# JackShDr/InfluentialRS

Hardware: AMD Instinct MI355X
Metric: scored user-item pairs/sec (whole node) (higher is better)
Workload: dtype f32; 1 GPU; c2: n_item=3415, d=128, L=200, H=4, layers=6, ffn=256; one greedy path-search step; users_per_gpu=4096, top_k=100, sweep=bf16 filter + exact f32 re-score, parallelism=single GPU

## Files before the change

### influentialrs_amd/csrc/decoder.hip

```cpp
#include "irs_internal.h"
#include "plane_split.h"

#include <assert.h>

typedef __attribute__((ext_vector_type(16))) float f32x16;

__global__ void __launch_bounds__(256) k_embed(const int64_t *__restrict__ seq, const float *__restrict__ E,
                                               const float *__restrict__ pe, float *__restrict__ x, int rows, int L,
                                               int d, float sqrtd, int64_t n_item) {
    int row = blockIdx.x * 4 + (threadIdx.x >> 6);
    int lane = threadIdx.x & 63;
    if (row >= rows) return;
    int64_t id = seq[row];
    if (id < 0) id = 0;
    if (id > n_item) id = n_item;
    int t = row % L;
    const float *e = E + id * (int64_t)d;
    const float *p = pe + (int64_t)t * d;
    float *o = x + (int64_t)row * d;
    for (int c = lane; c < d; c += 64) o[c] = __fadd_rn(__fmul_rn(e[c], sqrtd), p[c]);
}

__global__ void k_pif(const int64_t *__restrict__ user, const float *__restrict__ U, const float *__restrict__ w,
                      const float *__restrict__ b, float *__restrict__ r_u, int B, int ud, int64_t n_user) {
// ... 1386 lines not shown
    return;
#endif
#pragma unroll
    for (int j = 0; j < 8; ++j) {
        const float v = t[8 * s + j];
        const __bf16 h = (__bf16)v;
        const float r1 = v - (float)h;
        const __bf16 m = (__bf16)r1;
        const float r2 = r1 - (float)m;
        X[0][j] = h;
        X[1][j] = m;
        X[2][j] = (__bf16)r2;
    }
}

template <int B_, int E_, class Fn>
__device__ __forceinline__ void x6_static_for(Fn &&fn) {
    if constexpr (B_ < E_) {
        fn(std::integral_constant<int, B_>{});
        x6_static_for<B_ + 1, E_>(fn);
    }
}
template <int OFF>
__device__ __forceinline__ x6_u32x4 x6_rd(unsigned int base) {
    x6_u32x4 v;
    asm volatile("ds_read_b128 %0, %1 offset:%2" : "=v"(v) : "v"(base), "i"(OFF));
    return v;
}

template <int OFF>
__device__ __forceinline__ x6_u32x4 x6_gld(const void *p) {
    x6_u32x4 v;
    asm volatile("global_load_dwordx4 %0, %1, off offset:%2" : "=v"(v) : "v"(p), "i"(OFF) : "memory");
    return v;
}

__device__ __forceinline__ unsigned int x6_gld32(const void *p) {
    unsigned int v;
    asm volatile("global_load_dword %0, %1, off" : "=v"(v) : "v"(p) : "memory");
    return v;
}

__device__ __forceinline__ unsigned int x6_gld32_sync(const void *p) {
    unsigned int v;
    asm volatile("global_load_dword %0, %1, off\n\ts_waitcnt vmcnt(0)" : "=v"(v) : "v"(p) : "memory");
    return v;
}

template <int OFF>
__device__ __forceinline__ void x6_gst(void *p, x6_u32x4 v) {
    asm volatile("global_store_dwordx4 %0, %1, off offset:%2" :: "v"(p), "v"(v), "i"(OFF) : "memory");
}

template <int OFF>
__device__ __forceinline__ void x6_wr64(unsigned int addr, __attribute__((ext_vector_type(4))) _Float16 v) {
    asm volatile("ds_write_b64 %0, %1 offset:%2" :: "v"(addr), "v"(v), "i"(OFF));
}

template <int OFF>
__device__ __forceinline__ x6_u32x4 x6_rd_sync(unsigned int base) {
    x6_u32x4 v;
    asm volatile("ds_read_b128 %0, %1 offset:%2\n\ts_waitcnt lgkmcnt(0)" : "=v"(v) : "v"(base), "i"(OFF));
    return v;
}

struct SeqTarget {
    int seq;
    float k[8], v[8];
};
__device__ __forceinline__ unsigned int seq_diag_mask(int L, int qb, bool tgt, int pq) {
    unsigned int pm = 0;
    const int k0_ = 16 * qb;
    if (L <= k0_) return 0;
    if (L - k0_ < 16) pm = (0xFFFFu << (L - k0_)) & 0xFFFFu;
    if (tgt && L - 1 >= k0_ && L - 1 < k0_ + 16) pm |= 1u << (L - 1 - k0_);
    if (pq >= k0_ && pq < k0_ + 16) pm |= 1u << (pq - k0_);
    return pm;
}
__device__ __forceinline__ void seq_attn_block(const float *Ks, const char *Vp, int PL, int L, int qb, unsigned int pm_diag, float tgt_add,
                                               bool tgt_ok, int pq, const float *qscr, float4 *of, bool store, int seq, SeqTarget &tg);
#ifndef SEQ_EXP
#define SEQ_EXP 0
#endif
#define X6_SEQ_VECS (256 + 12 * 32 * 4 + 384)
#define X6_SEQ_KIMG (3 * 16384 + X6_SEQ_VECS * 4)
#define X6_SEQ_VIMG (X6_SEQ_KIMG + 32768)
#define X6_SEQ_SCR (X6_SEQ_VIMG + 32768)
#define X6_SEQ_SCR_B 4608
__host__ __device__ constexpr int x6_seq_lds_bytes() { return X6_SEQ_SCR + 8 * X6_SEQ_SCR_B; }
#ifdef X6_STAMP
#define X6_T(v_) { unsigned long long t_; asm volatile("s_memtime %0\n\ts_waitcnt lgkmcnt(0)" : "=s"(t_) :: "memory"); v_ = t_; }
#if X6_STAMP + 0 == 2
#define X6_TI(v_)
#else
#define X6_TI(v_) X6_T(v_)
#endif
#define X6_PH(i_) { unsigned long long t_; asm volatile("s_memtime %0\n\ts_waitcnt lgkmcnt(0)" : "=s"(t_) :: "memory"); st_ph[i_] += t_ - st_prev; st_prev = t_; }
#else
#define X6_T(v_)
#define X6_TI(v_)
#define X6_PH(i_)
#endif
template <int QP0, int NW, bool EMBED, int NT = 4, int NPL = 3, bool SEQ = false>
__global__ void __launch_bounds__(64 * NW, (NT == 8 || NW == 8) ? 1 : 2) k_block_x6(BlockX6Args a) {
    static_assert(!SEQ || (NT == 4 && NPL == 2 && NW == 8 && !EMBED && QP0 == 3), "the sequence-resident form: d = 128, float16 planes, eight waves, no q | k | v tail");
    constexpr int NP = 8 * NPL, STEP_B = x6_step_b(NPL);
    using x6_plane = typename std::conditional<NPL == 2, x6_f16x8, x6_bf16x8>::type;
    constexpr int D = 32 * NT, F = 256, NSLOT = SEQ ? 3 : x6_nslot(NPL), LEAD = NSLOT - 1, PPW = NP / NW, HT = NT / 4;
    constexpr int NFRONT = SEQ ? 3 * NT : 0;
    constexpr float WS = x6_wscale(NPL), IWS = 1.0f / WS;
    constexpr bool RESID_LATE = NPL == 2 && NT == 4 && !EMBED && NSLOT == 4 && (NW == 4 || NW == 8);
    constexpr bool RESID_SEP = RESID_LATE || SEQ;
    constexpr int NLOAD = 4 * NT;
    constexpr int NPRE = x6_npre(NT), NOUT = NT * HT;
    constexpr int S0 = EMBED ? NPRE : 0;
    constexpr int V_B1 = 0, V_B2 = F, V_G = F + D, V_B = F + 2 * D, V_BIN = F + 3 * D, V_O = F + 3 * D + 3 * D;
    constexpr int V_BQ = V_O + 6 * D;
    static_assert(NT == 4 || NT == 8, "d = 128 or 256");
    extern __shared__ __attribute__((aligned(16))) char smem[];
    float *vecs = reinterpret_cast<float *>(smem + NSLOT * STEP_B);
    const int tid = threadIdx.x;
    const int lane = tid & 63, wave = __builtin_amdgcn_readfirstlane(tid >> 6);
    const int li = lane & 31, lk = lane >> 5;
    unsigned long long st_p[8] = {0, 0, 0, 0, 0, 0, 0, 0};
    X6_T(st_p[0])
    const int m0 = blockIdx.x * (32 * NW);
    const int M = SEQ ? 0x7FFFFFFF : (a.m_dev ? min(a.M, a.m_dev[0]) : a.M);
    int sh_b[2] = {-1, -1}, sh_qb[2] = {0, 0}, sh_cnt[2] = {0, 0}, sh_pq[2] = {-1, -1}, sh_row0[2] = {0, 0};
    int sh_off[2] = {0, 0};
    float sh_ru[2] = {0.f, 0.f};
    bool sh_tgt[2] = {false, false};
    unsigned int sh_pm[2] = {0, 0};
    float sh_tadd[2] = {0.f, 0.f};
    if constexpr (SEQ) {
        if ((int)blockIdx.x >= a.n_wg_dev[0]) return;
        const int tg_ = blockIdx.x * NW + wave;
        const bool irn_ = a.mask_mode == IRS_MASK_IRN;
#pragma unroll
        for (int h = 0; h < 2; ++h) {
            const int b_ = __builtin_amdgcn_readfirstlane(a.tile_seq[2 * tg_ + h]);
            sh_b[h] = b_;
            if (b_ >= 0) {
                sh_qb[h] = __builtin_amdgcn_readfirstlane(a.tile_qb[2 * tg_ + h]);
                const int off_ = __builtin_amdgcn_readfirstlane(a.seq_off[b_]);
                sh_off[h] = off_;
                sh_cnt[h] = __builtin_amdgcn_readfirstlane(a.seq_cnt[b_]);
                sh_pq[h] = __builtin_amdgcn_readfirstlane(a.seq_padq[b_]), sh_row0[h] = __builtin_amdgcn_readfirstlane(a.seq_row0[b_]);
                sh_ru[h] = irn_ ? a.r_u[b_] : 0.f;
                sh_tgt[h] = irn_ && a.seq[(int64_t)b_ * a.L + a.L - 1] != 0;
                sh_pm[h] = seq_diag_mask(sh_cnt[h], sh_qb[h], sh_tgt[h], sh_pq[h]);
                sh_tadd[h] = __builtin_bit_cast(float, __builtin_amdgcn_readfirstlane(__builtin_bit_cast(int, irn_ ? (1.0f - sh_ru[h]) * 1.4426950408889634f : 0.f)));
            }
        }
    }
    float pv[RESID_LATE ? 13 : 1];
    if constexpr (RESID_LATE) {
        const int td = tid & (D - 1);
        const float *pbo = a.bo ? a.bo : a.b2, *pc = a.c ? a.c : a.b2, *pg2 = a.c ? a.g2 : a.b2, *pb2n = a.c ? a.b2n : a.b2;
        pv[0] = a.b1[tid], pv[1] = a.bin[tid], pv[2] = a.bin[256 + td], pv[3] = a.b2[td], pv[4] = a.g[td], pv[5] = a.b[td];
        pv[6] = pbo[td], pv[7] = a.g1[td], pv[8] = a.b1n[td], pv[9] = pc[td], pv[10] = pg2[td], pv[11] = pb2n[td];
        pv[12] = 0.f;
    }
    if (!SEQ && m0 >= M) return;
    if constexpr (RESID_LATE) {
        static_assert(NW == 4 || NW == 8, "every thread index below 256 exists");
        asm volatile("" ::"v"(pv[0]), "v"(pv[1]), "v"(pv[2]), "v"(pv[3]), "v"(pv[4]), "v"(pv[5]), "v"(pv[6]), "v"(pv[7]), "v"(pv[8]),
                     "v"(pv[9]), "v"(pv[10]), "v"(pv[11]));
        if (tid < 256) {
            vecs[V_B1 + tid] = pv[0];
            vecs[V_BIN + tid] = pv[1];
        }
        if (tid < D) {
            vecs[V_BIN + 256 + tid] = pv[2];
            vecs[V_B2 + tid] = pv[3], vecs[V_G + tid] = pv[4], vecs[V_B + tid] = pv[5];
            vecs[V_O + 0 * D + tid] = a.bo ? pv[6] : 0.f;
            vecs[V_O + 1 * D + tid] = pv[7];
            vecs[V_O + 2 * D + tid] = pv[8];
            vecs[V_O + 3 * D + tid] = a.c ? pv[9] : 0.f;
            vecs[V_O + 4 * D + tid] = a.c ? pv[10] : 0.f;
            vecs[V_O + 5 * D + tid] = a.c ? pv[11] : 0.f;
        }
    } else if constexpr (NT == 4) {
        if constexpr (SEQ) {
            constexpr int NV_ = (X6_SEQ_VECS + 64 * NW - 1) / (64 * NW);
// ... 200 lines not shown
#pragma unroll
            for (int tn = 0; tn < NT; ++tn)
#pragma unroll
                for (int g = 0; g < 4; ++g) {
                    const float4 t4 = rfrag[(tn * 4 + g) * 64];
                    acc[tn][4 * g + 0] = t4.x * WS, acc[tn][4 * g + 1] = t4.y * WS, acc[tn][4 * g + 2] = t4.z * WS, acc[tn][4 * g + 3] = t4.w * WS;
                }
        }
        if constexpr (RESID_LATE) {
            x6_static_for<0, NT>([&](auto tc) __attribute__((always_inline)) {
                constexpr int tn = decltype(tc)::value;
                const float4 *tp = afrag + tn * 4 * 64;
                atq[tn][0] = x6_gld<0>(tp), atq[tn][1] = x6_gld<1024>(tp), atq[tn][2] = x6_gld<2048>(tp), atq[tn][3] = x6_gld<3072>(tp);
            });
        } else if constexpr (!SEQ) {
#pragma unroll
            for (int tn = 0; tn < NT; ++tn)
#pragma unroll
                for (int g = 0; g < 4; ++g) {
                    const float4 t4 = afrag[(tn * 4 + g) * 64];
                    at[tn][4 * g + 0] = t4.x, at[tn][4 * g + 1] = t4.y, at[tn][4 * g + 2] = t4.z, at[tn][4 * g + 3] = t4.w;
                }
        }
        if constexpr (RESID_LATE) {
#pragma unroll
            for (int tn = 0; tn < NT; ++tn)
#pragma unroll
                for (int r = 0; r < 16; ++r) acc[tn][r] = 0.f;
        }
    } else {
        const int l31 = lane & 31, lhi = lane >> 5;
        char *scr = smem + wave * 16384;
        float4 *xo = reinterpret_cast<float4 *>(a.Xf) + fbase;
        int64_t rid[16];
        int rpos[16];
#pragma unroll
        for (int i = 0; i < 16; ++i) {
            const int mr = m0 + wave * 32 + 2 * i + lhi;
            const int orig = mr < M ? (a.tok_row ? a.tok_row[mr] : mr) : 0;
            int64_t id = mr < M ? a.seq[orig] : 0;
            if (id < 0) id = 0;
            if (id > a.n_item) id = a.n_item;
            rid[i] = id, rpos[i] = orig % a.L;
        }
#pragma unroll
        for (int hf = 0; hf < NT / 4; ++hf) {
            float4 ev[16], pv[16];
#pragma unroll
            for (int i = 0; i < 16; ++i) {
                ev[i] = *reinterpret_cast<const float4 *>(a.E + rid[i] * (int64_t)D + 128 * hf + 4 * l31);
                pv[i] = *reinterpret_cast<const float4 *>(a.pe + (int64_t)rpos[i] * D + 128 * hf + 4 * l31);
            }
#pragma unroll
            for (int i = 0; i < 16; ++i) {
                const int r = 2 * i + lhi;
                const bool live = m0 + wave * 32 + r < M;
                float4 v = make_float4(0.f, 0.f, 0.f, 0.f);
                if (live)
                    v = make_float4(__fadd_rn(__fmul_rn(ev[i].x, a.sqrtd), pv[i].x), __fadd_rn(__fmul_rn(ev[i].y, a.sqrtd), pv[i].y),
                                    __fadd_rn(__fmul_rn(ev[i].z, a.sqrtd), pv[i].z), __fadd_rn(__fmul_rn(ev[i].w, a.sqrtd), pv[i].w));
                *reinterpret_cast<float4 *>(scr + r * 512 + ((l31 ^ r) << 4)) = v;
            }
#pragma unroll
            for (int t4 = 0; t4 < 4; ++t4)
#pragma unroll
                for (int g = 0; g < 4; ++g) {
                    const int tn = 4 * hf + t4, c = 8 * t4 + 2 * g + lk;
                    const float4 v = *reinterpret_cast<const float4 *>(scr + li * 512 + ((c ^ li) << 4));
                    xo[(tn * 4 + g) * 64] = v;
                    acc[tn][4 * g + 0] = v.x, acc[tn][4 * g + 1] = v.y, acc[tn][4 * g + 2] = v.z, acc[tn][4 * g + 3] = v.w;
                }
        }
        __syncthreads();
    }
    auto load_res = [&]() __attribute__((always_inline)) {
        if constexpr (RESID_SEP) {
            const float4 *rfrag = reinterpret_cast<const float4 *>(a.Rf) + fbase;
            x6_static_for<0, NT>([&](auto tc) __attribute__((always_inline)) {
                constexpr int tn = decltype(tc)::value;
                const float4 *tp = rfrag + tn * 4 * 64;
                resq[tn][0] = x6_gld<0>(tp), resq[tn][1] = x6_gld<1024>(tp), resq[tn][2] = x6_gld<2048>(tp), resq[tn][3] = x6_gld<3072>(tp);
            });
        }
    };
    if constexpr (RESID_LATE) {
        asm volatile("s_waitcnt vmcnt(%0) lgkmcnt(0)" :: "i"(PPW * (LEAD - 1) + NLOAD) : "memory");
        __builtin_amdgcn_s_barrier();
    } else {
        issue(S0);
        asm volatile("s_waitcnt vmcnt(0) lgkmcnt(0)" ::: "memory");
        __builtin_amdgcn_s_barrier();
        x6_static_for<1, LEAD>([&](auto ic) __attribute__((always_inline)) { issue(S0 + decltype(ic)::value); });
    }

    constexpr int RING = 4, RA = RING - 1;
    static_assert(NP % RING == 0 && (NP + 8) % RING == 0 && RA <= NP / 2, "ring index continuity; next-step reads stay behind the barrier");
    x6_u32x4 af[RING];
    auto landed_all = [&]() __attribute__((always_inline)) {
#pragma unroll
        for (int q = 0; q < RING; ++q) asm volatile("s_waitcnt lgkmcnt(0)" : "+v"(af[q]));
    };
    x6_static_for<0, RING>([&](auto qc) __attribute__((always_inline)) {
        constexpr int q = decltype(qc)::value, off = (S0 % NSLOT) * STEP_B + (q < RA ? q : RA - 1) * 1024;
        if constexpr (NT == 8) af[q] = x6_rd_sync<off>(fr_addr);
        else af[q] = x6_rd<off>(fr_addr);
    });
    if constexpr (NT != 8) landed_all();

    auto seq_sync_tail = [&](int i) __attribute__((always_inline)) {
        return (i < NFRONT && i % 3 == 2) || i == NFRONT + NOUT - 1 || i == NFRONT + NPRE - 1;
    };
    const float invn = 1.0f / (float)D;
    x6_plane X[NPL];
    unsigned long long st_a = 0, st_b = 0, st_c = 0, st_d = 0, st_wait = 0, st_bar = 0, st_iss = 0, st_0 = 0, st_1 = 0, st_steps = 0;
    X6_T(st_0)
#ifdef X6_NO_MFMA
#define X6_MM(W_, X_, T_) { const auto mw_ = (W_); const auto mx_ = (X_); asm volatile("" :: "v"(mw_), "v"(mx_)); }
#else
#define X6_MM(W_, X_, T_) T_ = x6_mma(W_, X_, T_)
#endif
#define X6_MFMA(Wreg, Xp, T_) X6_MM(__builtin_bit_cast(x6_plane, Wreg), X[Xp], T_)
#ifdef X6_DUMP
#define X6_DUMP_FRAG(I_, f_) if (blockIdx.x == 0 && wave == 0) a.dbg[((I_) * NP + (f_)) * 64 + lane] = __builtin_bit_cast(uint4, af[(f_) & RA]);
#else
#define X6_DUMP_FRAG(I_, f_)
#endif
#ifdef X6_NO_READS
#define X6_READ_AHEAD(f_) asm volatile("" : "+v"(af[(f_) & RA]));
#else
#define X6_READ_AHEAD(f_)                                                                                                \
    if constexpr ((f_) + RA < NP) af[((f_) + RA) & RA] = x6_rd<((f_) + RA) * 1024>(sb_);                                 \
    else if (SEQ && !(SEQ_EXP & 2) && seq_sync_tail(step_)) af[((f_) + RA) & RA] = x6_rd_sync<((f_) + RA - NP) * 1024>(sn_);  \
    else af[((f_) + RA) & RA] = x6_rd<((f_) + RA - NP) * 1024>(sn_);  \
    asm volatile("s_waitcnt lgkmcnt(%1)" : "+v"(af[(f_) & RA]) : "i"(RA));                                               \
    X6_DUMP_FRAG(step_, f_)
#endif
#ifdef X6_NO_DMA
#define X6_ISSUE(i_)
#else
#define X6_ISSUE(i_) issue(i_)
#endif
#ifdef X6_NO_BARRIER
#define X6_PUBLISH(I_) if ((I_) + LEAD < nsteps) X6_ISSUE((I_) + LEAD);
#else
#define X6_PUBLISH(I_)                                                                                                   \
    if ((I_) + 1 < nsteps) {                                                                                             \
        X6_TI(st_a)                                                                                                       \
        if (RESID_LATE && (I_) < 4) asm volatile("s_waitcnt vmcnt(%0)" :: "i"(PPW * (LEAD - 2) + NLOAD) : "memory");  \
        else if (LEAD > 2 && (I_) + 2 < nsteps) asm volatile("s_waitcnt vmcnt(%0)" :: "i"(PPW * (LEAD - 2)) : "memory");      \
        else asm volatile("s_waitcnt vmcnt(0)" ::: "memory");                                                            \
        X6_TI(st_b)                                                                                                       \
        __builtin_amdgcn_s_barrier();                                                                                    \
        X6_TI(st_c)                                                                                                       \
        if ((I_) + LEAD < nsteps && !(SEQ && (I_) == NFRONT + NPRE - 1 && end_rt))  \
            X6_ISSUE((I_) + LEAD);                                                                                        \
        if constexpr (RESID_LATE) { if ((I_) == 1) load_res(); }                                                         \
        X6_TI(st_d)                                                                                                       \
        st_wait += st_b - st_a, st_bar += st_c - st_b, st_iss += st_d - st_c;                                            \
        if (SEQ && (I_) < NFRONT && (I_) % 3 == 0) st_ph[10] += st_c - st_b;  \
        if (SEQ && (I_) == NFRONT) st_ph[11] += st_c - st_b;                  \
    }
#endif
#define X6_STEP(I_, SRC, T0, T1, T2, T3)                                                                                \
    {                                                                                                                    \
        const int step_ = (I_);                                                                                          \
        unsigned long long sq_0 = 0, sq_1 = 0;                                                                           \
        X6_TI(sq_0)                                                                                                       \
        const unsigned int sb_ = fr_addr + (unsigned int)((step_ % NSLOT) * STEP_B);                                     \
        const unsigned int sn_ = fr_addr + (unsigned int)(((step_ + 1) % NSLOT) * STEP_B);                               \
        x6_static_for<0, NP>([&](auto fc_) __attribute__((always_inline)) {                                              \
            constexpr int f_ = decltype(fc_)::value, g_ = f_ / NPL, pl_ = f_ % NPL;                                      \
            if constexpr (f_ == 0) x6_split(SRC, 0, X);                                                                  \
            if constexpr (f_ == NP / 2) {                                                                                \
                X6_PUBLISH(step_)                                                                                        \
                x6_split(SRC, 1, X);                                                                                     \
            }                                                                                                            \
            X6_READ_AHEAD(f_)                                                                                            \
            f32x16 &T_ = (g_ & 3) == 0 ? T0 : (g_ & 3) == 1 ? T1 : (g_ & 3) == 2 ? T2 : T3;                              \
             \
            x6_static_for<0, NPL - pl_>([&](auto qc_) __attribute__((always_inline)) {                                   \
                X6_MFMA(af[f_ & RA], NPL - 1 - pl_ - decltype(qc_)::value, T_);                                           \
            });                                                                                                          \
        });                                                                                                              \
        X6_TI(sq_1)                                                                                                       \
        st_steps += sq_1 - sq_0;                                                                                         \
        __builtin_amdgcn_sched_barrier(0);                                                                               \
    }

    auto vec_stream = [&](auto na_c, auto o0_c, auto o1_c, auto o2_c, auto &&use) __attribute__((always_inline)) {
        constexpr int NA = decltype(na_c)::value, O0 = decltype(o0_c)::value, O1 = decltype(o1_c)::value, O2 = decltype(o2_c)::value;
        constexpr int NG = 4 * NT, AH = NA == 1 ? 3 : 2, RG = AH + 1;
        x6_u32x4 pr[RG][NA];
        auto rd = [&](auto gc) __attribute__((always_inline)) {
            constexpr int gi = decltype(gc)::value, goff = ((gi >> 2) * 32 + (gi & 3) * 8) * 4;
            pr[gi % RG][0] = x6_rd<O0 * 4 + goff>(vecs_addr);
            if constexpr (NA > 1) pr[gi % RG][1] = x6_rd<O1 * 4 + goff>(vecs_addr);
            if constexpr (NA > 2) pr[gi % RG][2] = x6_rd<O2 * 4 + goff>(vecs_addr);
        };
        x6_static_for<0, AH>(rd);
        x6_static_for<0, NG>([&](auto gc) __attribute__((always_inline)) {
            constexpr int gi = decltype(gc)::value, newer = NA * (gi + AH < NG ? AH : NG - 1 - gi);
            if constexpr (gi + AH < NG) rd(std::integral_constant<int, gi + AH>{});
            if constexpr (NA == 1) asm volatile("s_waitcnt lgkmcnt(%1)" : "+v"(pr[gi % RG][0]) : "i"(newer));
            if constexpr (NA == 2) asm volatile("s_waitcnt lgkmcnt(%2)" : "+v"(pr[gi % RG][0]), "+v"(pr[gi % RG][1]) : "i"(newer));
            if constexpr (NA == 3) asm volatile("s_waitcnt lgkmcnt(%3)" : "+v"(pr[gi % RG][0]), "+v"(pr[gi % RG][1]), "+v"(pr[gi % RG][2]) : "i"(newer));
            use(gc, __builtin_bit_cast(float4, pr[gi % RG][0]), __builtin_bit_cast(float4, pr[gi % RG][NA > 1 ? 1 : 0]),
                __builtin_bit_cast(float4, pr[gi % RG][NA > 2 ? 2 : 0]));
        });
    };
    constexpr bool ASM_VECS = NT == 4;
    using x6_ic0 = std::integral_constant<int, 0>;
    auto layer_norm = [&](auto vb_c, auto vg_c, auto vbeta_c, auto vadd_c) __attribute__((always_inline)) {
        constexpr int vb = decltype(vb_c)::value, vg = decltype(vg_c)::value, vbeta = decltype(vbeta_c)::value, vadd = decltype(vadd_c)::value;
        float sum = 0.f;
        if constexpr (ASM_VECS && vb >= 0) {
            vec_stream(std::integral_constant<int, 1>{}, vb_c, x6_ic0{}, x6_ic0{}, [&](auto gc, const float4 bb, const float4, const float4) __attribute__((always_inline)) {
                constexpr int tn = decltype(gc)::value >> 2, g = decltype(gc)::value & 3;
                if constexpr (RESID_SEP) {
                    const float4 rs = __builtin_bit_cast(float4, resq[tn][g]);
                    acc[tn][4 * g + 0] = __builtin_fmaf(acc[tn][4 * g + 0], IWS, rs.x), acc[tn][4 * g + 1] = __builtin_fmaf(acc[tn][4 * g + 1], IWS, rs.y);
                    acc[tn][4 * g + 2] = __builtin_fmaf(acc[tn][4 * g + 2], IWS, rs.z), acc[tn][4 * g + 3] = __builtin_fmaf(acc[tn][4 * g + 3], IWS, rs.w);
                    acc[tn][4 * g + 0] += bb.x, acc[tn][4 * g + 1] += bb.y, acc[tn][4 * g + 2] += bb.z, acc[tn][4 * g + 3] += bb.w;
                } else {
                    acc[tn][4 * g + 0] = __builtin_fmaf(acc[tn][4 * g + 0], IWS, bb.x), acc[tn][4 * g + 1] = __builtin_fmaf(acc[tn][4 * g + 1], IWS, bb.y);
                    acc[tn][4 * g + 2] = __builtin_fmaf(acc[tn][4 * g + 2], IWS, bb.z), acc[tn][4 * g + 3] = __builtin_fmaf(acc[tn][4 * g + 3], IWS, bb.w);
                }
                sum += (acc[tn][4 * g + 0] + acc[tn][4 * g + 1]) + (acc[tn][4 * g + 2] + acc[tn][4 * g + 3]);
            });
        } else {
#pragma unroll
            for (int tn = 0; tn < NT; ++tn)
#pragma unroll
                for (int g = 0; g < 4; ++g) {
                    if constexpr (vb >= 0) {
                        const float4 bb = *reinterpret_cast<const float4 *>(vecs + vb + tn * 32 + 8 * g + 4 * lk);
                        acc[tn][4 * g + 0] = __builtin_fmaf(acc[tn][4 * g + 0], IWS, bb.x), acc[tn][4 * g + 1] = __builtin_fmaf(acc[tn][4 * g + 1], IWS, bb.y);
                        acc[tn][4 * g + 2] = __builtin_fmaf(acc[tn][4 * g + 2], IWS, bb.z), acc[tn][4 * g + 3] = __builtin_fmaf(acc[tn][4 * g + 3], IWS, bb.w);
                    }
                    sum += (acc[tn][4 * g + 0] + acc[tn][4 * g + 1]) + (acc[tn][4 * g + 2] + acc[tn][4 * g + 3]);
                    if constexpr (!ASM_VECS) __builtin_amdgcn_sched_barrier(0);
                }
        }
        const float mu = lanes_sum<32>(sum) * invn;
        float qs = 0.f;
#pragma unroll
        for (int tn = 0; tn < NT; ++tn)
#pragma unroll
            for (int r = 0; r < 16; ++r) {
                const float dlt = acc[tn][r] - mu;
                qs += dlt * dlt;
            }
        const float rstd = 1.0f / sqrtf(lanes_sum<32>(qs) * invn + 1e-5f);
        if constexpr (ASM_VECS) {
            auto norm = [&](auto gc, const float4 gg, const float4 be, const float4 ad_) __attribute__((always_inline)) {
                constexpr int tn = decltype(gc)::value >> 2, g = decltype(gc)::value & 3;
                const float4 ad = vadd >= 0 ? ad_ : make_float4(0.f, 0.f, 0.f, 0.f);
                acc[tn][4 * g + 0] = (acc[tn][4 * g + 0] - mu) * rstd * gg.x + be.x + ad.x;
                acc[tn][4 * g + 1] = (acc[tn][4 * g + 1] - mu) * rstd * gg.y + be.y + ad.y;
                acc[tn][4 * g + 2] = (acc[tn][4 * g + 2] - mu) * rstd * gg.z + be.z + ad.z;
                acc[tn][4 * g + 3] = (acc[tn][4 * g + 3] - mu) * rstd * gg.w + be.w + ad.w;
// ... 104 lines not shown
    if constexpr (SEQ) {
        float *Kimg = reinterpret_cast<float *>(smem + X6_SEQ_KIMG);
        char *Vimg = smem + X6_SEQ_VIMG;
        float *scr = reinterpret_cast<float *>(smem + X6_SEQ_SCR + wave * X6_SEQ_SCR_B);
        int irow = l_row0 + s_j, li_l = li, sj_l = s_j;
        asm volatile("" : "+v"(irow), "+v"(li_l), "+v"(sj_l));
        const bool irn_ = a.mask_mode == IRS_MASK_IRN;
        float4 *ao4 = reinterpret_cast<float4 *>(const_cast<float *>(a.Af)) + (size_t)mtile * NT * 4 * 64;
#pragma unroll
        for (int h = 0; h < NT; ++h) {
            f32x16 tq, tk, tv, bt;
#pragma unroll
            for (int r = 0; r < 16; ++r) tq[r] = 0.f, tk[r] = 0.f, tv[r] = 0.f;
            x6_u32x4 rb;
            auto front_ride = [&](auto vc, auto cc, const f32x16 &t) __attribute__((always_inline)) {
                constexpr int v = decltype(vc)::value, c = decltype(cc)::value, g = v / 6;
                static_assert(NV == 24 && RA == 3, "a bias group every six reads, used three reads behind its own read");
                typedef __attribute__((ext_vector_type(4))) _Float16 f16x4;
                if constexpr (v % 6 == 0) rb = x6_rd<32 * g>(vecs_addr + (unsigned int)((V_BQ + c * D + 32 * h) * 4));
                if constexpr (v % 6 == 3) {
#ifdef X6_NO_READS
                    asm volatile("s_waitcnt lgkmcnt(0)" : "+v"(rb));
#else
                    asm volatile("s_waitcnt lgkmcnt(%1)" : "+v"(rb) : "i"(RA));
#endif
                    const float4 bb = __builtin_bit_cast(float4, rb);
                    const float bv[4] = {bb.x, bb.y, bb.z, bb.w};
                    f16x4 hp, lp;
                    const float x[4] = {__builtin_fmaf(t[4 * g], IWS, bv[0]), __builtin_fmaf(t[4 * g + 1], IWS, bv[1]),
                                        __builtin_fmaf(t[4 * g + 2], IWS, bv[2]), __builtin_fmaf(t[4 * g + 3], IWS, bv[3])};
#pragma unroll
                    for (int e = 0; e < 4; ++e) hp[e] = (_Float16)x[e];
                    irs_split_low(x, hp, lp);
                    if constexpr (c == 1) {
                        const int swk = (sj_l >> 1) & 7;
                        const unsigned int krow = lds0 + X6_SEQ_KIMG + (unsigned int)(irow * 128 + 8 * lk);
                        if (l_b >= 0) {
                            x6_wr64<0>(krow + ((g ^ swk) << 4), hp);
                            x6_wr64<0>(krow + (((4 + g) ^ swk) << 4), lp);
                        }
                    } else {
                        const int swv = ((sj_l >> 2) & 1) << 1;
                        const unsigned int slot = lds0 + X6_SEQ_VIMG + (unsigned int)(irow * 64 + ((g ^ swv) << 4) + 8 * lk);
                        if (l_b >= 0) {
                            x6_wr64<0>(slot, hp);
                            x6_wr64<16384>(slot, lp);
                        }
                    }
                }
            };
            auto ride_k = [&](auto vc) __attribute__((always_inline)) { front_ride(vc, std::integral_constant<int, 1>{}, tk); };
            auto ride_v = [&](auto vc) __attribute__((always_inline)) { front_ride(vc, std::integral_constant<int, 2>{}, tv); };
            X6_STEP1(3 * h, Yp, tk)
            X6_STEP1R(3 * h + 1, Yp, tv, ride_k)
            X6_STEP1R(3 * h + 2, Yp, tq, ride_v)
            X6_PH(9)
            bias_tile(bt, V_BQ + 32 * h);
            {
#pragma unroll
                for (int g = 0; g < 4; ++g)
                    *reinterpret_cast<float4 *>(scr + li_l * 36 + 8 * g + 4 * lk) =
                        make_float4(__builtin_fmaf(tq[4 * g + 0], IWS, bt[4 * g + 0]), __builtin_fmaf(tq[4 * g + 1], IWS, bt[4 * g + 1]),
                                    __builtin_fmaf(tq[4 * g + 2], IWS, bt[4 * g + 2]), __builtin_fmaf(tq[4 * g + 3], IWS, bt[4 * g + 3]));
            }
            asm volatile("s_waitcnt lgkmcnt(0)" ::: "memory");
            X6_PH(0)
            __builtin_amdgcn_s_barrier();
            asm volatile("" ::: "memory");
            X6_PH(1)
            if (!(SEQ_EXP & 1)) {
                SeqTarget tg;
                tg.seq = -1;
#pragma unroll 1
                for (int blk = 0; blk < 2; ++blk) {
                    const int b_ = blk ? sh_b[1] : sh_b[0], qb_ = blk ? sh_qb[1] : sh_qb[0], row0_ = blk ? sh_row0[1] : sh_row0[0];
                    seq_attn_block(Kimg + row0_ * 32, Vimg + row0_ * 64, 16384, b_ >= 0 ? (blk ? sh_cnt[1] : sh_cnt[0]) : 0, b_ >= 0 ? qb_ : 16,
                                   blk ? sh_pm[1] : sh_pm[0], blk ? sh_tadd[1] : sh_tadd[0], blk ? sh_tgt[1] : sh_tgt[0],
                                   blk ? sh_pq[1] : sh_pq[0], scr + 16 * blk * 36, ao4 + (size_t)h * 4 * 64 + 16 * blk, true, b_, tg);
                }
            }
            asm volatile("" ::: "memory");
            X6_PH(2)
        }
        __builtin_amdgcn_fence(__ATOMIC_SEQ_CST, "workgroup");
        {
            const float4 *afrag = reinterpret_cast<const float4 *>(a.Af) + fbase;
            x6_static_for<0, NT>([&](auto tc) __attribute__((always_inline)) {
                constexpr int tn = decltype(tc)::value;
                const float4 *tp = afrag + tn * 4 * 64;
                atq[tn][0] = x6_gld<0>(tp), atq[tn][1] = x6_gld<1024>(tp), atq[tn][2] = x6_gld<2048>(tp), atq[tn][3] = x6_gld<3072>(tp);
            });
            load_res();
            static_assert(NT == 4, "sixteen operands per statement");
            asm volatile("s_waitcnt vmcnt(0)"
                         : "+v"(atq[0][0]), "+v"(atq[0][1]), "+v"(atq[0][2]), "+v"(atq[0][3]), "+v"(atq[1][0]), "+v"(atq[1][1]), "+v"(atq[1][2]),
                           "+v"(atq[1][3]), "+v"(atq[2][0]), "+v"(atq[2][1]), "+v"(atq[2][2]), "+v"(atq[2][3]), "+v"(atq[3][0]), "+v"(atq[3][1]),
                           "+v"(atq[3][2]), "+v"(atq[3][3]));
            asm volatile("" : "+v"(resq[0][0]), "+v"(resq[0][1]), "+v"(resq[0][2]), "+v"(resq[0][3]), "+v"(resq[1][0]), "+v"(resq[1][1]),
                              "+v"(resq[1][2]), "+v"(resq[1][3]), "+v"(resq[2][0]), "+v"(resq[2][1]), "+v"(resq[2][2]), "+v"(resq[2][3]),
                              "+v"(resq[3][0]), "+v"(resq[3][1]), "+v"(resq[3][2]), "+v"(resq[3][3]));
#pragma unroll
            for (int tn = 0; tn < NT; ++tn)
#pragma unroll
                for (int g = 0; g < 4; ++g) {
                    const float4 u4 = __builtin_bit_cast(float4, atq[tn][g]);
                    at[tn][4 * g + 0] = u4.x, at[tn][4 * g + 1] = u4.y, at[tn][4 * g + 2] = u4.z, at[tn][4 * g + 3] = u4.w;
#pragma unroll
                    for (int e = 0; e < 4; ++e) acc[tn][4 * g + e] = 0.f;
                }
        }
        X6_PH(3)
    }
    if constexpr (!EMBED) {
#pragma unroll
        for (int t = 0; t < NT; ++t) {
            if constexpr (RESID_LATE) {
                const int newer_ = 4 * (NT - 1 - t) + PPW * t + (t >= 2 ? NLOAD : 0);
                asm volatile("s_waitcnt vmcnt(%4)" : "+v"(atq[t][0]), "+v"(atq[t][1]), "+v"(atq[t][2]), "+v"(atq[t][3]) : "n"(newer_));
#pragma unroll
                for (int g = 0; g < 4; ++g) {
                    const float4 t4 = __builtin_bit_cast(float4, atq[t][g]);
                    at[t][4 * g + 0] = t4.x, at[t][4 * g + 1] = t4.y, at[t][4 * g + 2] = t4.z, at[t][4 * g + 3] = t4.w;
                }
            }
            X6_STEP(NFRONT + t * HT, at[t], acc[0], acc[1], acc[2], acc[3])
            if constexpr (HT == 2) { X6_STEP(t * HT + 1, at[t], acc[4], acc[5], acc[6], acc[7]) }
        }
    }
    if constexpr (NT == 8) landed_all();
    X6_T(st_p[1])
    X6_PH(4)
    if constexpr (!EMBED) {
        using x6_icn = std::integral_constant<int, -1>;
        if constexpr (RESID_LATE) {
            static_assert(NT == 4, "sixteen operands");
            asm volatile("s_waitcnt vmcnt(%16)"
                         : "+v"(resq[0][0]), "+v"(resq[0][1]), "+v"(resq[0][2]), "+v"(resq[0][3]), "+v"(resq[1][0]), "+v"(resq[1][1]),
                           "+v"(resq[1][2]), "+v"(resq[1][3]), "+v"(resq[2][0]), "+v"(resq[2][1]), "+v"(resq[2][2]), "+v"(resq[2][3]),
                           "+v"(resq[3][0]), "+v"(resq[3][1]), "+v"(resq[3][2]), "+v"(resq[3][3])
                         : "n"(2 * PPW));
        }
        layer_norm(std::integral_constant<int, V_O + 0 * D>{}, std::integral_constant<int, V_O + 1 * D>{},
                   std::integral_constant<int, V_O + 2 * D>{}, std::integral_constant<int, V_O + 3 * D>{});
        if (a.c) layer_norm(x6_icn{}, std::integral_constant<int, V_O + 4 * D>{}, std::integral_constant<int, V_O + 5 * D>{}, x6_icn{});
    }
    X6_T(st_p[2])
    X6_PH(5)

    if constexpr (!EMBED) {
#pragma unroll
        for (int tn = 0; tn < NT; ++tn)
#pragma unroll
            for (int s2 = 0; s2 < 2; ++s2) {
                x6_split(acc[tn], s2, Yp[tn][s2]);
                __builtin_amdgcn_sched_barrier(0);
            }
        if constexpr (SEQ) {
#pragma unroll
            for (int k = 0; k < (X6_SEQ_VECS + 64 * NW - 1) / (64 * NW); ++k)
                nv[k] = (tid + 64 * NW * k < X6_SEQ_VECS) ? a.vecpack[(size_t)(ly + 1) * X6_SEQ_VECS + tid + 64 * NW * k] : 0.f;
        }
        if constexpr (NPL == 2) {
#pragma unroll
            for (int tn = 0; tn < NT; ++tn)
#pragma unroll
                for (int r = 0; r < 16; ++r) acc[tn][r] *= WS;
        }
    }
    if constexpr (!EMBED) {
#pragma unroll
        for (int ft = 0; ft < 8; ++ft) {
            f32x16 hft, bt;
#pragma unroll
            for (int r = 0; r < 16; ++r) hft[r] = 0.f;
            X6_STEP1(NFRONT + NOUT + 2 * HT * ft, Yp, hft)
            if constexpr (HT == 2) { X6_STEP1(NOUT + 4 * ft + 1, (&Yp[4]), hft) }
            bias_tile(bt, V_B1 + ft * 32);
#pragma unroll
            for (int r = 0; r < 16; ++r) hft[r] = fmaxf(__builtin_fmaf(hft[r], IWS, bt[r]), 0.f);
            X6_STEP(NFRONT + NOUT + 2 * HT * ft + HT, hft, acc[0], acc[1], acc[2], acc[3])
            if constexpr (HT == 2) { X6_STEP(NOUT + 4 * ft + 3, hft, acc[4], acc[5], acc[6], acc[7]) }
        }
    }
    if constexpr (NT == 8) landed_all();
    X6_T(st_p[3])
    X6_PH(6)
    if constexpr (!EMBED) {
        float sum = 0.f;
        if constexpr (ASM_VECS) {
            vec_stream(std::integral_constant<int, 1>{}, std::integral_constant<int, V_B2>{}, x6_ic0{}, x6_ic0{},
                       [&](auto gc, const float4 bb, const float4, const float4) __attribute__((always_inline)) {
                constexpr int tn = decltype(gc)::value >> 2, g = decltype(gc)::value & 3;
                acc[tn][4 * g + 0] = __builtin_fmaf(acc[tn][4 * g + 0], IWS, bb.x), acc[tn][4 * g + 1] = __builtin_fmaf(acc[tn][4 * g + 1], IWS, bb.y);
                acc[tn][4 * g + 2] = __builtin_fmaf(acc[tn][4 * g + 2], IWS, bb.z), acc[tn][4 * g + 3] = __builtin_fmaf(acc[tn][4 * g + 3], IWS, bb.w);
                sum += (acc[tn][4 * g + 0] + acc[tn][4 * g + 1]) + (acc[tn][4 * g + 2] + acc[tn][4 * g + 3]);
            });
        } else {
#pragma unroll
        for (int tn = 0; tn < NT; ++tn)
#pragma unroll
            for (int g = 0; g < 4; ++g) {
                const float4 bb = *reinterpret_cast<const float4 *>(vecs + V_B2 + tn * 32 + 8 * g + 4 * lk);
                acc[tn][4 * g + 0] = __builtin_fmaf(acc[tn][4 * g + 0], IWS, bb.x), acc[tn][4 * g + 1] = __builtin_fmaf(acc[tn][4 * g + 1], IWS, bb.y);
                acc[tn][4 * g + 2] = __builtin_fmaf(acc[tn][4 * g + 2], IWS, bb.z), acc[tn][4 * g + 3] = __builtin_fmaf(acc[tn][4 * g + 3], IWS, bb.w);
                sum += (acc[tn][4 * g + 0] + acc[tn][4 * g + 1]) + (acc[tn][4 * g + 2] + acc[tn][4 * g + 3]);
                __builtin_amdgcn_sched_barrier(0);
            }
        }
        const float mu = lanes_sum<32>(sum) * invn;
        float qs = 0.f;
#pragma unroll
        for (int tn = 0; tn < NT; ++tn)
#pragma unroll
            for (int r = 0; r < 16; ++r) {
                const float dlt = acc[tn][r] - mu;
                qs += dlt * dlt;
            }
        const float rstd = 1.0f / sqrtf(lanes_sum<32>(qs) * invn + 1e-5f);
        if constexpr (ASM_VECS) {
            char *xt = nullptr;
            if constexpr (SEQ) {
                int mt_ = (int)blockIdx.x * NW + wave;
                asm volatile("" : "+s"(mt_));
                xt = reinterpret_cast<char *>(a.Xf) + ((size_t)mt_ * (4 * NT) * 64 + lane) * 16;
            }
            vec_stream(std::integral_constant<int, 2>{}, std::integral_constant<int, V_G>{}, std::integral_constant<int, V_B>{}, x6_ic0{},
                       [&](auto gc, const float4 gg, const float4 be, const float4) __attribute__((always_inline)) {
                constexpr int tn = decltype(gc)::value >> 2, g = decltype(gc)::value & 3;
                const float4 o = make_float4((acc[tn][4 * g + 0] - mu) * rstd * gg.x + be.x, (acc[tn][4 * g + 1] - mu) * rstd * gg.y + be.y,
                                             (acc[tn][4 * g + 2] - mu) * rstd * gg.z + be.z, (acc[tn][4 * g + 3] - mu) * rstd * gg.w + be.w);
                if constexpr (SEQ) x6_gst<1024 * g>(xt + 4096 * tn, __builtin_bit_cast(x6_u32x4, o));
                else if (a.Xf) reinterpret_cast<float4 *>(a.Xf)[((size_t)(mtile * NT + tn) * 4 + g) * 64 + lane] = o;
                acc[tn][4 * g + 0] = o.x, acc[tn][4 * g + 1] = o.y, acc[tn][4 * g + 2] = o.z, acc[tn][4 * g + 3] = o.w;
            });
        } else {
#pragma unroll
        for (int tn = 0; tn < NT; ++tn)
#pragma unroll
            for (int g = 0; g < 4; ++g) {
                const int n = tn * 32 + 8 * g + 4 * lk;
                const float4 gg = *reinterpret_cast<const float4 *>(vecs + V_G + n);
                const float4 be = *reinterpret_cast<const float4 *>(vecs + V_B + n);
                const float4 o = make_float4((acc[tn][4 * g + 0] - mu) * rstd * gg.x + be.x, (acc[tn][4 * g + 1] - mu) * rstd * gg.y + be.y,
                                             (acc[tn][4 * g + 2] - mu) * rstd * gg.z + be.z, (acc[tn][4 * g + 3] - mu) * rstd * gg.w + be.w);
                if (a.Xf) reinterpret_cast<float4 *>(a.Xf)[((size_t)(mtile * NT + tn) * 4 + g) * 64 + lane] = o;
                acc[tn][4 * g + 0] = o.x, acc[tn][4 * g + 1] = o.y, acc[tn][4 * g + 2] = o.z, acc[tn][4 * g + 3] = o.w;
                __builtin_amdgcn_sched_barrier(0);
            }
        }
    }
#pragma unroll
    for (int tn = 0; tn < NT; ++tn)
#pragma unroll
        for (int s2 = 0; s2 < 2; ++s2) {
            x6_split(acc[tn], s2, Yp[tn][s2]);
            __builtin_amdgcn_sched_barrier(0);
        }
    X6_T(st_p[4])
    X6_PH(7)
    if (SEQ && end_rt) return;
    if (SEQ) {
        asm volatile("s_waitcnt vmcnt(0)" ::: "memory");
        __builtin_amdgcn_s_barrier();
        asm volatile("" ::: "memory");
#pragma unroll
        for (int k = 0; k < (X6_SEQ_VECS + 64 * NW - 1) / (64 * NW); ++k)
            if (tid + 64 * NW * k < X6_SEQ_VECS) vecs[tid + 64 * NW * k] = nv[k];
        asm volatile("s_waitcnt lgkmcnt(0)" ::: "memory");
        issue(SEQ_LSTEPS - 1 + LEAD);
        af[0] = x6_rd_sync<0>(fr_addr), af[1] = x6_rd_sync<1024>(fr_addr), af[2] = x6_rd_sync<2048>(fr_addr);
        X6_PH(8)
        return;
    }
#pragma unroll
    for (int pp = 0; pp < 3; ++pp) {
        if (pp >= 3 - QP0) break;
        const int c0 = D * (pp + QP0);
#pragma unroll
        for (int i = 0; i < NT; ++i) {
            f32x16 qt, bt;
#pragma unroll
            for (int r = 0; r < 16; ++r) qt[r] = 0.f;
            X6_STEP1(NFRONT + NPRE + HT * (NT * pp + i), Yp, qt)
            if constexpr (HT == 2) { X6_STEP1(NPRE + 2 * (NT * pp + i) + 1, (&Yp[4]), qt) }
            bias_tile(bt, V_BIN + c0 + i * 32);
            X6_T(st_q0)
#ifdef X6_NO_QKV_STORE
            asm volatile("" :: "v"(qt[0]), "v"(qt[5]), "v"(qt[10]), "v"(qt[15]), "v"(bt[0]));
            if (mt < M && a.M < 0) {
#else
            if (mt < M) {
#endif
                float *qrow = a.QKV + (int64_t)mt * (3 * D) + c0 + i * 32 + 4 * lk;
                if (QP0 == 0 && a.kv_planes && pp == 2) {
                    typedef __attribute__((ext_vector_type(4))) _Float16 f16x4;
                    char *slot = reinterpret_cast<char *>(a.QKV + (int64_t)mt * (3 * D) + c0 + i * 32) + 8 * lk;
#pragma unroll
                    for (int g = 0; g < 4; ++g) {
                        f16x4 hp, lp;
                        const float v[4] = {__builtin_fmaf(qt[4 * g], IWS, bt[4 * g]), __builtin_fmaf(qt[4 * g + 1], IWS, bt[4 * g + 1]),
                                            __builtin_fmaf(qt[4 * g + 2], IWS, bt[4 * g + 2]), __builtin_fmaf(qt[4 * g + 3], IWS, bt[4 * g + 3])};
#pragma unroll
                        for (int e = 0; e < 4; ++e) hp[e] = (_Float16)v[e];
                        irs_split_low(v, hp, lp);
                        *reinterpret_cast<f16x4 *>(slot + 16 * g) = hp;
                        *reinterpret_cast<f16x4 *>(slot + 64 + 16 * g) = lp;
                    }
                } else {
#pragma unroll
                    for (int g = 0; g < 4; ++g)
                        *reinterpret_cast<float4 *>(qrow + 8 * g) =
                            make_float4(__builtin_fmaf(qt[4 * g + 0], IWS, bt[4 * g + 0]), __builtin_fmaf(qt[4 * g + 1], IWS, bt[4 * g + 1]),
                                        __builtin_fmaf(qt[4 * g + 2], IWS, bt[4 * g + 2]), __builtin_fmaf(qt[4 * g + 3], IWS, bt[4 * g + 3]));
                }
            }
            X6_T(st_q1)
            st_qst += st_q1 - st_q0;
        }
    }
    };
    if constexpr (SEQ) {
#pragma unroll 1
        for (ly = 0; ly < a.n_lay; ++ly) layer_body();
    } else
        layer_body();
    landed_all();
    if constexpr (SEQ) asm volatile("s_waitcnt vmcnt(0)" ::: "memory");
#ifdef X6_STAMP
    X6_T(st_1)
    if (lane == 0 && a.stamps) {
        unsigned long long *o = a.stamps + (size_t)(blockIdx.x * NW + wave) * (SEQ ? 24 : 8);
        if constexpr (SEQ) {
#pragma unroll
            for (int i = 0; i < 12; ++i) o[8 + i] = st_ph[i];
        }
        o[0] = st_1 - st_p[0], o[1] = st_wait, o[2] = st_bar, o[3] = st_iss, o[4] = st_steps;
        o[5] = st_0 - st_p[0];
        o[6] = (st_p[2] - st_p[1]) + (st_p[4] - st_p[3]);
        o[7] = st_qst;
    }
#endif
    (void)st_ph, (void)st_prev;
    (void)st_p, (void)st_q0, (void)st_q1, (void)st_qst;
    (void)st_a, (void)st_b, (void)st_c, (void)st_d, (void)st_wait, (void)st_bar, (void)st_iss, (void)st_0, (void)st_1, (void)st_steps;
#undef nsteps
#undef last
#undef X6_STEP
#undef X6_STEP1
#undef X6_STEP1R
#undef X6_RD_V
#undef X6_WAIT_V
#undef X6_PUBLISH
#undef X6_ISSUE
#undef X6_READ_AHEAD
#undef X6_MFMA
#undef X6_MM
}

struct EmbedQkvArgs {
    const int64_t *seq;
    const float *E, *pe;
    const int32_t *tok_row, *m_dev;
    int rows, L;
    float sqrtd;
    int64_t n_item;
    float *Xf;
    const float *Win, *bin;
    float *QKV;
};

__global__ void __launch_bounds__(256, 2) k_embed_qkv(EmbedQkvArgs a) {
    constexpr int D = 128, BK = 16, NR = 192;
    __shared__ __attribute__((aligned(16))) float sm[2 * NR * BK + 3 * D];
    float *vb = sm + 2 * NR * BK;
    const int tid = threadIdx.x, lane = tid & 63, wave = tid >> 6;
    const int li = lane & 31, lk = lane >> 5;
    const int m0 = blockIdx.x * 128;
    const int M = a.m_dev ? min(a.rows, a.m_dev[0]) : a.rows;
    if (m0 >= M) return;
    vb[tid] = a.bin[tid];
    if (tid < D) vb[256 + tid] = a.bin[256 + tid];
    const int mtile = (m0 >> 5) + wave;
    const int mt = m0 + wave * 32 + li;
    const bool live = mt < M;
    float4 wv[3];
    auto load_slab = [&](int t) {
        const int pp = t >> 3, ss = t & 7;
#pragma unroll
        for (int i = 0; i < 3; ++i) {
            const int idx = tid + i * 256;
            const float *p = a.Win + (size_t)(NR * pp + (idx >> 2)) * D + ss * BK + (idx & 3) * 4;
            wv[i] = make_float4(p[0], p[1], p[2], p[3]);
        }
    };
    auto store_slab = [&](float *S) {
#pragma unroll
        for (int i = 0; i < 3; ++i) {
            const int idx = tid + i * 256;
            const int r = idx >> 2, c = idx & 3;
            *reinterpret_cast<float4 *>(S + r * BK + ((c ^ lin_swz<BK>(r)) << 2)) = wv[i];
        }
    };
    load_slab(0);
    f32x16 acc[4];
    {
        const int orig = live ? (a.tok_row ? a.tok_row[mt] : mt) : 0;
        int64_t id = live ? a.seq[orig] : 0;
        if (id < 0) id = 0;
        if (id > a.n_item) id = a.n_item;
        const float *e = a.E + id * (int64_t)D;
// ... 3618 lines not shown
```

### influentialrs_amd/csrc/irs_internal.h

```cpp
#pragma once

#include <hip/hip_runtime.h>
#include <stdint.h>
#include <stdio.h>
#include <string.h>

#include "../../include/irs_hip.h"

#if !defined(IRS_LAB) && (defined(X6_DUMP) || defined(X6_STAMP) || defined(X6_NO_SPLIT) || defined(X6_NO_MFMA) ||            \
                          defined(X6_NO_READS) || defined(X6_NO_DMA) || defined(X6_NO_BARRIER) || defined(X6_NO_QKV_STORE) ||  \
                          defined(X6_NW) || defined(SEQ_EXP) || defined(PLAN_STAMP) || defined(ATTN_STAMP) ||                  \
                          defined(IRS_SMALL_TIMING) || defined(IRS_DIRECT_TIMING))
#error "a lab switch (X6_* / SEQ_EXP / *_STAMP / IRS_*_TIMING) is defined without IRS_LAB: the product library must be built without them"
#endif

#include <atomic>
#include <functional>
#define IRS_MAX_DEVICES 32
static inline int irs_cur_dev() {
    int d = 0;
    if (hipGetDevice(&d) != hipSuccess || d < 0 || d >= IRS_MAX_DEVICES) d = 0;
    return d;
}
#define IRS_ONCE_PER_DEVICE(body_)                                                                                        \
    do {                                                                                                                  \
        static std::atomic<unsigned> once_mask_{0};                                                                       \
        const unsigned once_bit_ = 1u << irs_cur_dev();                                                                   \
        if (!(once_mask_.load(std::memory_order_acquire) & once_bit_)) {                                                  \
            body_;                                                                                                        \
            once_mask_.fetch_or(once_bit_, std::memory_order_release);                                                    \
        }                                                                                                                 \
    } while (0)

#define IRS_MAX_LAYERS 16
#define IRS_CAND_BUCKETS 64
#define IRS_CAND_SLOTS 64
#define IRS_CAND_CAP (IRS_CAND_BUCKETS * IRS_CAND_SLOTS)
#define IRS_REFINE_CAP 1024
#define IRS_MAX_GROUPS 2048
#define IRS_MAX_PATH 64
#define IRS_MAX_EXCL 4096
#define IRS_LSE_SLOTS_RING 4096
#define IRS_COOP_FALLBACK_MIN_ITEMS 262144
#define IRS_EXH_SCRATCH_KEYS (64 * 32768)

struct irs_layer_w {
    const float *sa_in_w, *sa_in_b, *sa_out_w, *sa_out_b;
    const float *ca_in_w, *ca_in_b, *ca_out_w, *ca_out_b;
    const float *l1_w, *l1_b, *l2_w, *l2_b;
    const float *n1_w, *n1_b, *n2_w, *n2_b, *n3_w, *n3_b;
};

struct irs_prof_ev {
    hipEvent_t a, b;
};

enum { IRS_STEP_GREEDY = 1, IRS_STEP_BEAM, IRS_STEP_SHARDED_BEAM, IRS_STEP_SHARDED_BEAM_SPLIT };
struct irs_step_key {
    int32_t kind, B, W, P, k, sweep, sample, sample_k;
    uint64_t seed;
    const void *comm, *seq, *user, *hep, *paths, *status;
    const void *tr_item, *tr_target, *tr_rank, *tr_scratch;
    int32_t arr_rank;
    uint32_t arr_lp_bits;
};
static_assert(sizeof(irs_step_key) == 8 * sizeof(int32_t) + 11 * 8 + 2 * sizeof(int32_t), "irs_step_key is compared with memcmp: no padding");
struct irs_step_graph {
    hipGraphExec_t exec;
    irs_step_key key;
};

struct irs_excl {
    const int64_t *rows;
    const int32_t *cnt;
    const int32_t *map;
    const float *paths;
    const int32_t *step_ptr;
    int stride, div;
    int path_ld, path_by_user;
    int step_arg, on;
};

struct irs_beam_state {
    int64_t *seq;
    int32_t *hep;
    double *cum;
    float *paths;
    int32_t *fin;
};
struct irs_beam_side {
    int64_t *user;
    int32_t *done;
    int32_t *map;
};
// ... 593 lines not shown
```

Measured before the change: 2.459 billion pairs/s.

## Relax vmcnt waits in sequence-resident layer loop and overlap residual loads

In the sequence-resident decoder block kernel, residual fragment loads are spread across the first weight step's fragments instead of being issued in one batch at the layer seam. The blocking vmcnt(0) waits are replaced with partial counts so the attention-output tiles and residuals are waited on one at a time. The store-side waits also leave the newest loads in flight. The seam fence is narrowed from workgroup to wavefront scope. The intent is to overlap global-memory latency with MFMA work. The vmcnt arithmetic is fragile, and a wrong count would let data be consumed before it has arrived.

```diff
diff --git a/influentialrs_amd/csrc/decoder.hip b/influentialrs_amd/csrc/decoder.hip
--- a/influentialrs_amd/csrc/decoder.hip
+++ b/influentialrs_amd/csrc/decoder.hip
@@ -1492,6 +1492,11 @@
 #ifndef SEQ_EXP
 #define SEQ_EXP 0
 #endif
+#ifndef SEQ_ACKS
+#define SEQ_ACKS 3
+#endif
+#define SEQ_TILE_WAITS ((SEQ_ACKS & 1) != 0)
+#define SEQ_STORE_WAITS ((SEQ_ACKS & 2) != 0)
 #define X6_SEQ_VECS (256 + 12 * 32 * 4 + 384)
 #define X6_SEQ_KIMG (3 * 16384 + X6_SEQ_VECS * 4)
 #define X6_SEQ_VIMG (X6_SEQ_KIMG + 32768)
@@ -1506,10 +1511,16 @@
 #define X6_TI(v_) X6_T(v_)
 #endif
 #define X6_PH(i_) { unsigned long long t_; asm volatile("s_memtime %0\n\ts_waitcnt lgkmcnt(0)" : "=s"(t_) :: "memory"); st_ph[i_] += t_ - st_prev; st_prev = t_; }
+#if X6_STAMP + 0 == 2
+#define X6_PH_SEAM X6_PH(10)
+#else
+#define X6_PH_SEAM
+#endif
 #else
 #define X6_T(v_)
 #define X6_TI(v_)
 #define X6_PH(i_)
+#define X6_PH_SEAM
 #endif
 template <int QP0, int NW, bool EMBED, int NT = 4, int NPL = 3, bool SEQ = false>
 __global__ void __launch_bounds__(64 * NW, (NT == 8 || NW == 8) ? 1 : 2) k_block_x6(BlockX6Args a) {
@@ -1876,6 +1887,11 @@
                 resq[tn][0] = x6_gld<0>(tp), resq[tn][1] = x6_gld<1024>(tp), resq[tn][2] = x6_gld<2048>(tp), resq[tn][3] = x6_gld<3072>(tp);
             });
         }
+    };
+    auto load_res_piece = [&](auto fc) __attribute__((always_inline)) {
+        constexpr int f = decltype(fc)::value;
+        static_assert(NP == 4 * NT || !SEQ, "a residual piece per fragment of the step");
+        if constexpr (SEQ) resq[f >> 2][f & 3] = x6_gld<1024 * (f & 3)>(reinterpret_cast<const float4 *>(a.Rf) + fbase + (f >> 2) * 4 * 64);
     };
     if constexpr (RESID_LATE) {
         asm volatile("s_waitcnt vmcnt(%0) lgkmcnt(0)" :: "i"(PPW * (LEAD - 1) + NLOAD) : "memory");
@@ -1941,6 +1957,8 @@
     if ((I_) + 1 < nsteps) {                                                                                             \
         X6_TI(st_a)                                                                                                       \
         if (RESID_LATE && (I_) < 4) asm volatile("s_waitcnt vmcnt(%0)" :: "i"(PPW * (LEAD - 2) + NLOAD) : "memory");  \
+        else if (SEQ && SEQ_TILE_WAITS && (I_) == NFRONT) asm volatile("s_waitcnt vmcnt(%0)" :: "i"(4 * (NT - 1) + NP / 2) : "memory");  \
+        else if (SEQ && SEQ_TILE_WAITS && (I_) == NFRONT + 1) asm volatile("s_waitcnt vmcnt(%0)" :: "i"(NP / 2) : "memory");  \
         else if (LEAD > 2 && (I_) + 2 < nsteps) asm volatile("s_waitcnt vmcnt(%0)" :: "i"(PPW * (LEAD - 2)) : "memory");      \
         else asm volatile("s_waitcnt vmcnt(0)" ::: "memory");                                                            \
         X6_TI(st_b)                                                                                                       \
@@ -1970,6 +1988,7 @@
                 x6_split(SRC, 1, X);                                                                                     \
             }                                                                                                            \
             X6_READ_AHEAD(f_)                                                                                            \
+            if constexpr (SEQ && SEQ_TILE_WAITS) { if (step_ == NFRONT) load_res_piece(fc_); }                           \
             f32x16 &T_ = (g_ & 3) == 0 ? T0 : (g_ & 3) == 1 ? T1 : (g_ & 3) == 2 ? T2 : T3;                              \
              \
             x6_static_for<0, NPL - pl_>([&](auto qc_) __attribute__((always_inline)) {                                   \
@@ -2240,7 +2259,10 @@
             asm volatile("" ::: "memory");
             X6_PH(2)
         }
-        __builtin_amdgcn_fence(__ATOMIC_SEQ_CST, "workgroup");
+        if constexpr (SEQ_ACKS == 0) __builtin_amdgcn_fence(__ATOMIC_SEQ_CST, "workgroup");
+        else __builtin_amdgcn_fence(__ATOMIC_SEQ_CST, "wavefront");
+        asm volatile("" ::: "memory");
+        X6_PH_SEAM
         {
             const float4 *afrag = reinterpret_cast<const float4 *>(a.Af) + fbase;
             x6_static_for<0, NT>([&](auto tc) __attribute__((always_inline)) {
@@ -2248,21 +2270,25 @@
                 const float4 *tp = afrag + tn * 4 * 64;
                 atq[tn][0] = x6_gld<0>(tp), atq[tn][1] = x6_gld<1024>(tp), atq[tn][2] = x6_gld<2048>(tp), atq[tn][3] = x6_gld<3072>(tp);
             });
-            load_res();
             static_assert(NT == 4, "sixteen operands per statement");
-            asm volatile("s_waitcnt vmcnt(0)"
-                         : "+v"(atq[0][0]), "+v"(atq[0][1]), "+v"(atq[0][2]), "+v"(atq[0][3]), "+v"(atq[1][0]), "+v"(atq[1][1]), "+v"(atq[1][2]),
-                           "+v"(atq[1][3]), "+v"(atq[2][0]), "+v"(atq[2][1]), "+v"(atq[2][2]), "+v"(atq[2][3]), "+v"(atq[3][0]), "+v"(atq[3][1]),
-                           "+v"(atq[3][2]), "+v"(atq[3][3]));
-            asm volatile("" : "+v"(resq[0][0]), "+v"(resq[0][1]), "+v"(resq[0][2]), "+v"(resq[0][3]), "+v"(resq[1][0]), "+v"(resq[1][1]),
-                              "+v"(resq[1][2]), "+v"(resq[1][3]), "+v"(resq[2][0]), "+v"(resq[2][1]), "+v"(resq[2][2]), "+v"(resq[2][3]),
-                              "+v"(resq[3][0]), "+v"(resq[3][1]), "+v"(resq[3][2]), "+v"(resq[3][3]));
+            if constexpr (!SEQ_TILE_WAITS) {
+                load_res();
+                asm volatile("s_waitcnt vmcnt(0)"
+                             : "+v"(atq[0][0]), "+v"(atq[0][1]), "+v"(atq[0][2]), "+v"(atq[0][3]), "+v"(atq[1][0]), "+v"(atq[1][1]), "+v"(atq[1][2]),
+                               "+v"(atq[1][3]), "+v"(atq[2][0]), "+v"(atq[2][1]), "+v"(atq[2][2]), "+v"(atq[2][3]), "+v"(atq[3][0]), "+v"(atq[3][1]),
+                               "+v"(atq[3][2]), "+v"(atq[3][3]));
+                asm volatile("" : "+v"(resq[0][0]), "+v"(resq[0][1]), "+v"(resq[0][2]), "+v"(resq[0][3]), "+v"(resq[1][0]), "+v"(resq[1][1]),
+                                  "+v"(resq[1][2]), "+v"(resq[1][3]), "+v"(resq[2][0]), "+v"(resq[2][1]), "+v"(resq[2][2]), "+v"(resq[2][3]),
+                                  "+v"(resq[3][0]), "+v"(resq[3][1]), "+v"(resq[3][2]), "+v"(resq[3][3]));
+            }
 #pragma unroll
             for (int tn = 0; tn < NT; ++tn)
 #pragma unroll
                 for (int g = 0; g < 4; ++g) {
-                    const float4 u4 = __builtin_bit_cast(float4, atq[tn][g]);
-                    at[tn][4 * g + 0] = u4.x, at[tn][4 * g + 1] = u4.y, at[tn][4 * g + 2] = u4.z, at[tn][4 * g + 3] = u4.w;
+                    if constexpr (!SEQ_TILE_WAITS) {
+                        const float4 u4 = __builtin_bit_cast(float4, atq[tn][g]);
+                        at[tn][4 * g + 0] = u4.x, at[tn][4 * g + 1] = u4.y, at[tn][4 * g + 2] = u4.z, at[tn][4 * g + 3] = u4.w;
+                    }
 #pragma unroll
                     for (int e = 0; e < 4; ++e) acc[tn][4 * g + e] = 0.f;
                 }
@@ -2272,8 +2298,8 @@
     if constexpr (!EMBED) {
 #pragma unroll
         for (int t = 0; t < NT; ++t) {
-            if constexpr (RESID_LATE) {
-                const int newer_ = 4 * (NT - 1 - t) + PPW * t + (t >= 2 ? NLOAD : 0);
+            if constexpr (RESID_LATE || (SEQ && SEQ_TILE_WAITS)) {
+                const int newer_ = 4 * (NT - 1 - t) + PPW * t + (t >= (SEQ ? 1 : 2) ? NLOAD : 0);
                 asm volatile("s_waitcnt vmcnt(%4)" : "+v"(atq[t][0]), "+v"(atq[t][1]), "+v"(atq[t][2]), "+v"(atq[t][3]) : "n"(newer_));
 #pragma unroll
                 for (int g = 0; g < 4; ++g) {
@@ -2290,13 +2316,13 @@
     X6_PH(4)
     if constexpr (!EMBED) {
         using x6_icn = std::integral_constant<int, -1>;
-        if constexpr (RESID_LATE) {
+        if constexpr (RESID_LATE || (SEQ && SEQ_TILE_WAITS)) {
             static_assert(NT == 4, "sixteen operands");
             asm volatile("s_waitcnt vmcnt(%16)"
                          : "+v"(resq[0][0]), "+v"(resq[0][1]), "+v"(resq[0][2]), "+v"(resq[0][3]), "+v"(resq[1][0]), "+v"(resq[1][1]),
                            "+v"(resq[1][2]), "+v"(resq[1][3]), "+v"(resq[2][0]), "+v"(resq[2][1]), "+v"(resq[2][2]), "+v"(resq[2][3]),
                            "+v"(resq[3][0]), "+v"(resq[3][1]), "+v"(resq[3][2]), "+v"(resq[3][3])
-                         : "n"(2 * PPW));
+                         : "n"(SEQ ? (NOUT - 1) * PPW : 2 * PPW));
         }
         layer_norm(std::integral_constant<int, V_O + 0 * D>{}, std::integral_constant<int, V_O + 1 * D>{},
                    std::integral_constant<int, V_O + 2 * D>{}, std::integral_constant<int, V_O + 3 * D>{});
@@ -2418,7 +2444,8 @@
     X6_PH(7)
     if (SEQ && end_rt) return;
     if (SEQ) {
-        asm volatile("s_waitcnt vmcnt(0)" ::: "memory");
+        if constexpr (SEQ_STORE_WAITS) asm volatile("s_waitcnt vmcnt(%0)" :: "i"(NLOAD) : "memory");
+        else asm volatile("s_waitcnt vmcnt(0)" ::: "memory");
         __builtin_amdgcn_s_barrier();
         asm volatile("" ::: "memory");
 #pragma unroll
@@ -2483,7 +2510,8 @@
     } else
         layer_body();
     landed_all();
-    if constexpr (SEQ) asm volatile("s_waitcnt vmcnt(0)" ::: "memory");
+    if constexpr (SEQ && SEQ_STORE_WAITS) asm volatile("s_waitcnt vmcnt(%0)" :: "i"(NLOAD) : "memory");
+    else if constexpr (SEQ) asm volatile("s_waitcnt vmcnt(0)" ::: "memory");
 #ifdef X6_STAMP
     X6_T(st_1)
     if (lane == 0 && a.stamps) {
diff --git a/influentialrs_amd/csrc/irs_internal.h b/influentialrs_amd/csrc/irs_internal.h
--- a/influentialrs_amd/csrc/irs_internal.h
+++ b/influentialrs_amd/csrc/irs_internal.h
@@ -9,7 +9,7 @@
 
 #if !defined(IRS_LAB) && (defined(X6_DUMP) || defined(X6_STAMP) || defined(X6_NO_SPLIT) || defined(X6_NO_MFMA) ||            \
                           defined(X6_NO_READS) || defined(X6_NO_DMA) || defined(X6_NO_BARRIER) || defined(X6_NO_QKV_STORE) ||  \
-                          defined(X6_NW) || defined(SEQ_EXP) || defined(PLAN_STAMP) || defined(ATTN_STAMP) ||                  \
+                          defined(X6_NW) || defined(SEQ_EXP) || defined(SEQ_ACKS) || defined(PLAN_STAMP) || defined(ATTN_STAMP) ||                  \
                           defined(IRS_SMALL_TIMING) || defined(IRS_DIRECT_TIMING))
 #error "a lab switch (X6_* / SEQ_EXP / *_STAMP / IRS_*_TIMING) is defined without IRS_LAB: the product library must be built without them"
 #endif
```

New measurement: 2.468 billion pairs/s, median of 6. No clear change (+0.4%).
